# hao-ai-lab/LookaheadDecoding

Measured on NVIDIA H100. Metric: tokens/sec (wall-clock) and accepted-tokens/step, Llama-2-7B W=15 N=5 G=15, higher is better.
Workload: dtype bf16

## Files before the change

### lookaheaddecoding_b200/csrc/attn_mma.cu

```cuda
#include "common.cuh"

namespace lade {

constexpr int ATT_BM = 128;
constexpr int ATT_BN = 64;
constexpr int ATT_STAGES = 3;
constexpr int ATT_THREADS = 256;
constexpr int ATT_RD_SMEM = 1024;
constexpr int ATTN_MAX_COUNTERS = 16384;

__device__ __forceinline__ void cp_async16(void* smem, const void* gmem, int src_bytes) {
  const unsigned s = (unsigned)__cvta_generic_to_shared(smem);
  asm volatile("cp.async.cg.shared.global [%0], [%1], 16, %2;\n" ::"r"(s), "l"(gmem), "r"(src_bytes));
}
__device__ __forceinline__ void cp_async_commit() { asm volatile("cp.async.commit_group;\n" ::); }
template <int N>
__device__ __forceinline__ void cp_async_wait() { asm volatile("cp.async.wait_group %0;\n" ::"n"(N)); }

__device__ __forceinline__ void ldmatrix_x4(unsigned& r0, unsigned& r1, unsigned& r2, unsigned& r3, const void* p) {
  const unsigned a = (unsigned)__cvta_generic_to_shared(p);
  asm volatile("ldmatrix.sync.aligned.m8n8.x4.shared.b16 {%0,%1,%2,%3}, [%4];\n"
               : "=r"(r0), "=r"(r1), "=r"(r2), "=r"(r3) : "r"(a));
}
__device__ __forceinline__ void ldmatrix_x4_trans(unsigned& r0, unsigned& r1, unsigned& r2, unsigned& r3, const void* p) {
  const unsigned a = (unsigned)__cvta_generic_to_shared(p);
  asm volatile("ldmatrix.sync.aligned.m8n8.x4.trans.shared.b16 {%0,%1,%2,%3}, [%4];\n"
               : "=r"(r0), "=r"(r1), "=r"(r2), "=r"(r3) : "r"(a));
}
template <typename T>
__device__ __forceinline__ void mma_16816(float (&c)[4], const unsigned (&a)[4], unsigned b0, unsigned b1);
template <>
__device__ __forceinline__ void mma_16816<__nv_bfloat16>(float (&c)[4], const unsigned (&a)[4], unsigned b0, unsigned b1) {
// ... 314 lines not shown
```

### lookaheaddecoding_b200/csrc/attn_tc.cu

```cuda
#include "tc_common.cuh"

#include <cstdlib>
#include <mutex>
#include <type_traits>
#include <unordered_map>

namespace lade {

constexpr int TC_BM = 128;
constexpr int TC_BN = 128;
constexpr int TC_D = 128;
constexpr int TC_STAGES = 3;
constexpr int TC_CONSUMER_THREADS = 256;
constexpr int TC_THREADS = TC_CONSUMER_THREADS + 32;
constexpr int TC_TILE_BYTES = 128 * 128 * 2;
constexpr int TC_HALF_BYTES = TC_TILE_BYTES / 2;
constexpr int TC_SMEM_TILES = TC_TILE_BYTES * (1 + 2 * TC_STAGES);
constexpr int TC_SMEM_BYTES = TC_SMEM_TILES + 256 + 1024;
constexpr float TC_LOG2E = 1.4426950408889634f;
constexpr int TC_SO_STRIDE = 132;
constexpr int TC_SO_OFFSET = TC_TILE_BYTES;
constexpr int TC_SML_OFFSET = 0;

__device__ long long* g_attn_timing = nullptr;
#define TC_STAMP(slot, tid) do { if (tbuf && threadIdx.x == (tid)) tbuf[slot] = clock64(); } while (0)
enum { TS_START = 0, TS_KFULL0 = 1, TS_SFULL0 = 2, TS_OFINAL = 3, TS_STAGED = 4, TS_CLUSTER = 5, TS_MERGED = 6, TS_END = 7 };

template <typename ET> __device__ __forceinline__ float2 unpack2(uint32_t u);
template <> __device__ __forceinline__ float2 unpack2<__nv_bfloat16>(uint32_t u) {
  return make_float2(__uint_as_float(u << 16), __uint_as_float(u & 0xffff0000u));
}
template <> __device__ __forceinline__ float2 unpack2<__half>(uint32_t u) {
  return __half22float2(*reinterpret_cast<__half2*>(&u));
}

template <typename ET>
__device__ __forceinline__ void qk_tile(float (&s)[64], uint32_t sQ_a, uint32_t sK_a, int wg) {
  wg_fence();
#pragma unroll
  for (int kb = 0; kb < 2; ++kb)
#pragma unroll
    for (int k = 0; k < 4; ++k) {
      const uint64_t da = wg_desc(sQ_a + kb * TC_HALF_BYTES + wg * 8192 + k * 32, 16, 1024);
      const uint64_t db = wg_desc(sK_a + kb * TC_HALF_BYTES + k * 32, 16, 1024);
      wgmma_m64n128_ss<ET>(s, da, db, (kb | k) ? 1u : 0u);
    }
  wg_commit();
  wg_wait_all();
  wg_fence_regs(s);
// ... 9 lines not shown
  wg_wait_all();
  wg_fence_regs(o);
}

__device__ __forceinline__ void tile_mask(uint32_t (&mb)[2][4], const uint32_t* const (&mrow)[2], const int (&row)[2],
                                          int mask_words, int tile0, int kv_len, int q_len, int is_prefill) {
#pragma unroll
  for (int rr = 0; rr < 2; ++rr)
#pragma unroll
    for (int w = 0; w < 4; ++w)
      mb[rr][w] = (tile0 + 32 * w + 32 <= kv_len)
                      ? 0xffffffffu
                      : visible_bits32(mrow[rr], mask_words, tile0 + 32 * w, kv_len, q_len, is_prefill, row[rr]);
}
__device__ __forceinline__ bool vis(const uint32_t (&mb)[2][4], int rr, int i, int e, int t) {
  return (mb[rr][i >> 2] >> (8 * (i & 3) + 2 * t + e)) & 1u;
}

template <typename ET, bool REF>
__global__ void __launch_bounds__(TC_THREADS, 1)
attn_fwd_tc_kernel(const __grid_constant__ CUtensorMap tmQ, const __grid_constant__ CUtensorMap tmK,
                   const __grid_constant__ CUtensorMap tmV, ET* __restrict__ out,
                   const uint32_t* __restrict__ rowmask, int mask_words, const int* __restrict__ meta, int q_pad,
                   int n_heads, int n_kv_heads, int n_splits, float inv_sqrt_d, float2* __restrict__ row_ml) {
  extern __shared__ unsigned char smem_raw[];
  const uint32_t raw_a = smem_u32(smem_raw);
  const uint32_t sQ_a = (raw_a + 1023u) & ~1023u;
  unsigned char* smem = smem_raw + (sQ_a - raw_a);
  const int split = blockIdx.x, h = blockIdx.y, mt = blockIdx.z;
  const int warp = threadIdx.x >> 5, lane = threadIdx.x & 31;

  const int q_len = meta[LADE_M_Q_LEN];
  const int kv_len = meta[LADE_M_KV_LEN];
  const int is_prefill = meta[LADE_M_IS_PREFILL];
  const int T = kv_len + q_len;
  int Tm = T;
  if (is_prefill) Tm = min(T, kv_len + min(q_len, (mt + 1) * TC_BM));
  const int n_tiles = (Tm + TC_BN - 1) / TC_BN;
  const int t_base = n_tiles / n_splits, t_rem = n_tiles - t_base * n_splits;
  const int n_active = n_tiles < n_splits ? n_tiles : n_splits;
  const bool active = split < n_active;
  const int tile_lo = split * t_base + (split < t_rem ? split : t_rem);
  const int my_tiles = active ? t_base + (split < t_rem ? 1 : 0) : 0;
  if (REF && t_base + (t_rem ? 1 : 0) > TC_STAGES) __trap();
  const int hk = h / (n_heads / n_kv_heads);
  const int HD = n_heads * TC_D;
  const long long hm = (long long)h * gridDim.z + mt;
  const int n_wg = (mt * TC_BM + 64 < q_pad) ? 2 : 1;
  const bool zero_last = active && (tile_lo + my_tiles) * TC_BN > T;
  long long* tbuf = g_attn_timing ? g_attn_timing + 16ll * ((blockIdx.z * gridDim.y + blockIdx.y) * gridDim.x + blockIdx.x) : nullptr;
  TC_STAMP(TS_START, 0);
  griddep_launch_dependents();

  uint64_t* bars = reinterpret_cast<uint64_t*>(smem + TC_SMEM_TILES);
  const uint32_t bar0 = smem_u32(bars);
  auto BAR = [&](int i) { return bar0 + 8u * (uint32_t)i; };
  const int B_QFULL = 0, B_KFULL = 1, B_VFULL = 1 + TC_STAGES, B_FREE = 1 + 2 * TC_STAGES, B_VZERO = 1 + 3 * TC_STAGES;
  auto sK_a = [&](int s) { return sQ_a + (uint32_t)TC_TILE_BYTES * (1 + 2 * s); };
  auto sV_a = [&](int s) { return sQ_a + (uint32_t)TC_TILE_BYTES * (2 + 2 * s); };
  auto issue_tile = [&](int j) {
    const int s = j % TC_STAGES;
    const int row0 = (tile_lo + j) * TC_BN;
    mbar_expect_tx(BAR(B_KFULL + s), TC_TILE_BYTES);
    tma_load_3d(sK_a(s), &tmK, BAR(B_KFULL + s), 0, row0, hk);
    tma_load_3d(sK_a(s) + TC_HALF_BYTES, &tmK, BAR(B_KFULL + s), 64, row0, hk);
    mbar_expect_tx(BAR(B_VFULL + s), TC_TILE_BYTES);
    tma_load_3d(sV_a(s), &tmV, BAR(B_VFULL + s), 0, row0, hk);
    tma_load_3d(sV_a(s) + TC_HALF_BYTES, &tmV, BAR(B_VFULL + s), 64, row0, hk);
  };

  if (active && threadIdx.x == TC_CONSUMER_THREADS) {
    mbar_init(BAR(B_QFULL), 1);
    for (int s = 0; s < TC_STAGES; ++s) {
      mbar_init(BAR(B_KFULL + s), 1);
      mbar_init(BAR(B_VFULL + s), 1);
      mbar_init(BAR(B_FREE + s), 4 * n_wg);
    }
    mbar_init(BAR(B_VZERO), 1);
    fence_barrier_init();
    const int n_pre = my_tiles < TC_STAGES ? my_tiles : TC_STAGES;
    int n_old = 0;
    while (n_old < n_pre && (tile_lo + n_old + 1) * TC_BN <= kv_len) ++n_old;
    for (int j = 0; j < n_old; ++j) issue_tile(j);
    griddep_wait();
    mbar_expect_tx(BAR(B_QFULL), TC_TILE_BYTES);
    tma_load_3d(sQ_a, &tmQ, BAR(B_QFULL), 0, mt * TC_BM, h);
    tma_load_3d(sQ_a + TC_HALF_BYTES, &tmQ, BAR(B_QFULL), 64, mt * TC_BM, h);
    for (int j = n_old; j < n_pre; ++j) issue_tile(j);
  }
  __syncthreads();

  const int wg = warp >> 2;
  const int g = lane >> 2, t = lane & 3;
  const int rl[2] = {wg * 64 + (warp & 3) * 16 + g, wg * 64 + (warp & 3) * 16 + g + 8};
  const bool work = active && warp < 8 && wg < n_wg;
  float o[64];
  float m_row[2] = {-INFINITY, -INFINITY}, l_row[2] = {0.f, 0.f};
#pragma unroll
  for (int i = 0; i < 64; ++i) o[i] = 0.f;

  if (warp == 8) {
    if (active) {
      if (lane == 0) {
        for (int j = TC_STAGES; j < my_tiles; ++j) {
          const int s = j % TC_STAGES;
          mbar_wait(BAR(B_FREE + s), ((j / TC_STAGES) - 1) & 1);
          issue_tile(j);
        }
      }
      __syncwarp();
      if (zero_last) {
        const int j = my_tiles - 1, s = j % TC_STAGES;
        const int r0 = T - (tile_lo + j) * TC_BN;
        mbar_wait(BAR(B_VFULL + s), (j / TC_STAGES) & 1);
        unsigned char* pV = smem + TC_TILE_BYTES * (2 + 2 * s);
        const uint4 z = make_uint4(0, 0, 0, 0);
        for (int c = r0 * 8 + lane; c < TC_BN * 8; c += 32) {
          const int r = c >> 3, cc = c & 7;
          *reinterpret_cast<uint4*>(pV + r * 128 + cc * 16) = z;
          *reinterpret_cast<uint4*>(pV + TC_HALF_BYTES + r * 128 + cc * 16) = z;
        }
        fence_proxy_async();
        __syncwarp();
        if (lane == 0) mbar_arrive(BAR(B_VZERO));
      }
    }
    if (REF) {
      cluster_arrive(); cluster_wait();
      cluster_arrive(); cluster_wait();
    }
  } else {
    const int row[2] = {mt * TC_BM + rl[0], mt * TC_BM + rl[1]};
    const uint32_t* const mrow[2] = {
        (row[0] < q_pad && !is_prefill && rowmask != nullptr) ? rowmask + (long long)row[0] * mask_words : nullptr,
        (row[1] < q_pad && !is_prefill && rowmask != nullptr) ? rowmask + (long long)row[1] * mask_words : nullptr};
    auto wait_v = [&](int j) {
      const int s = j % TC_STAGES;
      mbar_wait(BAR(B_VFULL + s), (j / TC_STAGES) & 1);
      if (zero_last && j == my_tiles - 1) mbar_wait(BAR(B_VZERO), 0);
    };
    if (work) mbar_wait(BAR(B_QFULL), 0);
    if (!REF) {
      for (int j = 0; work && j < my_tiles; ++j) {
        const int s = j % TC_STAGES;
        const int tile0 = (tile_lo + j) * TC_BN;
        mbar_wait(BAR(B_KFULL + s), (j / TC_STAGES) & 1);
        if (j == 0) TC_STAMP(TS_KFULL0, 0);
        float sc[64];
        qk_tile<ET>(sc, sQ_a, sK_a(s), wg);
        if (j == 0) TC_STAMP(TS_SFULL0, 0);
        uint32_t mb[2][4];
        tile_mask(mb, mrow, row, mask_words, tile0, kv_len, q_len, is_prefill);
        float off[2];
#pragma unroll
        for (int rr = 0; rr < 2; ++rr) {
          float mx = -INFINITY;
#pragma unroll
          for (int i = 0; i < 16; ++i)
#pragma unroll
            for (int e = 0; e < 2; ++e) mx = fmaxf(mx, vis(mb, rr, i, e, t) ? sc[4 * i + 2 * rr + e] : -INFINITY);
          mx = fmaxf(mx, __shfl_xor_sync(0xffffffffu, mx, 1));
          mx = fmaxf(mx, __shfl_xor_sync(0xffffffffu, mx, 2));
          const float mtile = mx == -INFINITY ? -INFINITY : round_to<ET>(round_to<ET>(mx) * inv_sqrt_d);
          if (mtile > m_row[rr]) {
            const float scale = m_row[rr] == -INFINITY ? 1.f : exp2f((m_row[rr] - mtile) * TC_LOG2E);
            l_row[rr] *= scale;
#pragma unroll
            for (int i = 0; i < 16; ++i) { o[4 * i + 2 * rr] *= scale; o[4 * i + 2 * rr + 1] *= scale; }
            m_row[rr] = mtile;
// ... 9 lines not shown
            round_scale_round2<ET>(sc[4 * i + 2 * rr], sc[4 * i + 2 * rr + 1], inv_sqrt_d, r0, r1);
            const float p0 = vis(mb, rr, i, 0, t) ? ex2_approx(r0 * TC_LOG2E - off[rr]) : 0.f;
            const float p1 = vis(mb, rr, i, 1, t) ? ex2_approx(r1 * TC_LOG2E - off[rr]) : 0.f;
            const uint32_t pk = Elem<ET>::pack2(p0, p1);
            const float2 pr = unpack2<ET>(pk);
            l_row[rr] += pr.x + pr.y;
            pa[4 * (i >> 1) + 2 * (i & 1) + rr] = pk;
          }
        wait_v(j);
        pv_tile<ET>(o, pa, sV_a(s));
        __syncwarp();
        if (lane == 0) mbar_arrive(BAR(B_FREE + s));
      }
#pragma unroll
      for (int rr = 0; rr < 2; ++rr) {
        l_row[rr] += __shfl_xor_sync(0xffffffffu, l_row[rr], 1);
        l_row[rr] += __shfl_xor_sync(0xffffffffu, l_row[rr], 2);
      }
    } else {
      float sc[64];
      uint32_t mb[2][4];
      float mx[2] = {-INFINITY, -INFINITY};
      for (int j = 0; work && j < my_tiles; ++j) {
        mbar_wait(BAR(B_KFULL + j), 0);
        qk_tile<ET>(sc, sQ_a, sK_a(j), wg);
        tile_mask(mb, mrow, row, mask_words, (tile_lo + j) * TC_BN, kv_len, q_len, is_prefill);
#pragma unroll
        for (int rr = 0; rr < 2; ++rr)
#pragma unroll
          for (int i = 0; i < 16; ++i)
#pragma unroll
            for (int e = 0; e < 2; ++e) mx[rr] = fmaxf(mx[rr], vis(mb, rr, i, e, t) ? sc[4 * i + 2 * rr + e] : -INFINITY);
      }
      if (work) {
#pragma unroll
        for (int rr = 0; rr < 2; ++rr) {
          mx[rr] = fmaxf(mx[rr], __shfl_xor_sync(0xffffffffu, mx[rr], 1));
          mx[rr] = fmaxf(mx[rr], __shfl_xor_sync(0xffffffffu, mx[rr], 2));
          const float m_split = mx[rr] == -INFINITY ? -INFINITY : round_to<ET>(round_to<ET>(mx[rr]) * inv_sqrt_d);
          if (t == 0) row_ml[(hm * n_splits + split) * TC_BM + rl[rr]].x = m_split;
        }
      }
      cluster_arrive(); cluster_wait();
      float m_ref[2] = {0.f, 0.f};
      if (work) {
#pragma unroll
        for (int rr = 0; rr < 2; ++rr) {
// ... 37 lines not shown
      }
      cluster_arrive(); cluster_wait();
      float l_all[2] = {0.f, 0.f};
      if (work) {
#pragma unroll
        for (int rr = 0; rr < 2; ++rr)
          for (int sp = 0; sp < n_active; ++sp) l_all[rr] += ld_global_f2(row_ml + (hm * n_splits + sp) * TC_BM + rl[rr]).y;
      }
      for (int j = 0; work && j < my_tiles; ++j) {
        exps(j);
        uint32_t pa[32];
#pragma unroll
        for (int i = 0; i < 16; ++i)
#pragma unroll
          for (int rr = 0; rr < 2; ++rr) {
            const float p0 = l_all[rr] > 0.f ? __fdiv_rn(sc[4 * i + 2 * rr], l_all[rr]) : 0.f;
            const float p1 = l_all[rr] > 0.f ? __fdiv_rn(sc[4 * i + 2 * rr + 1], l_all[rr]) : 0.f;
            pa[4 * (i >> 1) + 2 * (i & 1) + rr] = Elem<ET>::pack2(p0, p1);
          }
        wait_v(j);
        pv_tile<ET>(o, pa, sV_a(j));
      }
    }
    TC_STAMP(TS_OFINAL, 0);
    if (work && n_splits == 1) {
#pragma unroll
      for (int rr = 0; rr < 2; ++rr) {
        if (row[rr] >= q_pad) continue;
        const float inv = REF ? 1.f : (l_row[rr] > 0.f ? 1.f / l_row[rr] : 0.f);
        uint32_t* dst = reinterpret_cast<uint32_t*>(out + (long long)row[rr] * HD + h * TC_D + 2 * t);
#pragma unroll
        for (int i = 0; i < 16; ++i) dst[4 * i] = Elem<ET>::pack2(o[4 * i + 2 * rr] * inv, o[4 * i + 2 * rr + 1] * inv);
      }
    }
  }
  TC_STAMP(TS_STAGED, 0);
  if (n_splits == 1) { TC_STAMP(TS_END, 0); return; }

  const int rows_valid = min(TC_BM, q_pad - mt * TC_BM);
  const int per = (rows_valid + n_active - 1) / n_active;
  cluster_arrive();
  cluster_wait();
  TC_STAMP(TS_CLUSTER, 0);
  int dest[2] = {-1, -1}, r_in[2] = {0, 0};
  if (work) {
#pragma unroll
    for (int rr = 0; rr < 2; ++rr) {
      dest[rr] = rl[rr] < rows_valid ? rl[rr] / per : -2;
      r_in[rr] = rl[rr] - dest[rr] * per;
      if (dest[rr] >= 0 && dest[rr] != split) {
        const int slot = split < dest[rr] ? split : split - 1;
        const uint32_t o_a = dsmem_addr(sQ_a + TC_SO_OFFSET + (uint32_t)(((slot * per + r_in[rr]) * TC_SO_STRIDE + 2 * t) * 4), dest[rr]);
#pragma unroll
        for (int i = 0; i < 16; ++i) st_dsmem_f2(o_a + i * 32, o[4 * i + 2 * rr], o[4 * i + 2 * rr + 1]);
        if (!REF && t == 0)
          st_dsmem_f2(dsmem_addr(sQ_a + TC_SML_OFFSET + (uint32_t)((slot * per + r_in[rr]) * 8), dest[rr]), m_row[rr], l_row[rr]);
      }
    }
  }
  cluster_arrive();
  cluster_wait();
  TC_STAMP(TS_MERGED, 0);
  if (work) {
    const float2* sml = reinterpret_cast<const float2*>(smem + TC_SML_OFFSET);
    const float* so = reinterpret_cast<const float*>(smem + TC_SO_OFFSET);
#pragma unroll
    for (int rr = 0; rr < 2; ++rr) {
      if (dest[rr] != split) continue;
      float inv = 1.f;
      if (!REF) {
        float mmax = m_row[rr];
        for (int k = 0; k < n_active - 1; ++k) mmax = fmaxf(mmax, sml[k * per + r_in[rr]].x);
        float wgt = (m_row[rr] == -INFINITY) ? 0.f : exp2f((m_row[rr] - mmax) * TC_LOG2E);
        float lsum = l_row[rr] * wgt;
#pragma unroll
        for (int i = 0; i < 16; ++i) { o[4 * i + 2 * rr] *= wgt; o[4 * i + 2 * rr + 1] *= wgt; }
        for (int k = 0; k < n_active - 1; ++k) {
          const float2 ml = sml[k * per + r_in[rr]];
          wgt = (ml.x == -INFINITY) ? 0.f : exp2f((ml.x - mmax) * TC_LOG2E);
          lsum += ml.y * wgt;
          const float* src = so + (k * per + r_in[rr]) * TC_SO_STRIDE + 2 * t;
#pragma unroll
          for (int i = 0; i < 16; ++i) {
            const float2 x = *reinterpret_cast<const float2*>(src + 8 * i);
            o[4 * i + 2 * rr] += x.x * wgt;
            o[4 * i + 2 * rr + 1] += x.y * wgt;
          }
        }
        inv = lsum > 0.f ? 1.f / lsum : 0.f;
      } else {
        for (int k = 0; k < n_active - 1; ++k) {
          const float* src = so + (k * per + r_in[rr]) * TC_SO_STRIDE + 2 * t;
#pragma unroll
          for (int i = 0; i < 16; ++i) {
            const float2 x = *reinterpret_cast<const float2*>(src + 8 * i);
            o[4 * i + 2 * rr] += x.x;
            o[4 * i + 2 * rr + 1] += x.y;
          }
        }
      }
      const int row = mt * TC_BM + rl[rr];
      if (row < q_pad) {
        uint32_t* dst = reinterpret_cast<uint32_t*>(out + (long long)row * HD + h * TC_D + 2 * t);
#pragma unroll
        for (int i = 0; i < 16; ++i) dst[4 * i] = Elem<ET>::pack2(o[4 * i + 2 * rr] * inv, o[4 * i + 2 * rr + 1] * inv);
      }
    }
  }
  TC_STAMP(TS_END, 0);
}

int attn_tc_set_timing_buffer(void* dev_ptr) {
  long long* p = reinterpret_cast<long long*>(dev_ptr);
  cudaError_t e = cudaMemcpyToSymbol(g_attn_timing, &p, sizeof(p));
  if (e != cudaSuccess) { set_cuda_error(e, "cudaMemcpyToSymbol(g_attn_timing)"); return LADE_ECUDA; }
  return LADE_OK;
}

EncodeTiledFn get_encode_fn() {
  static EncodeTiledFn fn = nullptr;
  static bool tried = false;
  if (!tried) {
    tried = true;
    void* p = nullptr;
    cudaDriverEntryPointQueryResult qres;
    if (cudaGetDriverEntryPoint("cuTensorMapEncodeTiled", &p, cudaEnableDefault, &qres) == cudaSuccess &&
        qres == cudaDriverEntryPointSuccess)
      fn = reinterpret_cast<EncodeTiledFn>(p);
  }
  return fn;
}

// ... 44 lines not shown
  return v != 0;
}

template <typename ET, bool REF>
static int launch_tc(cudaStream_t stream, const void* q, const void* k_cache, const void* v_cache, void* out,
                     const uint32_t* rowmask, int mask_words, const int32_t* meta, void* scratch, int q_pad, int n_heads,
                     int n_kv_heads, int head_dim, int kv_capacity, int n_splits) {
  const int q_tiles = (q_pad + TC_BM - 1) / TC_BM;
  if ((reinterpret_cast<uintptr_t>(q) & 15) || (reinterpret_cast<uintptr_t>(k_cache) & 15) ||
      (reinterpret_cast<uintptr_t>(v_cache) & 15))
    return LADE_EINVAL;
  CUtensorMap tmQ, tmK, tmV;
  int rc;
  if ((rc = get_tensor_map(q, q_pad, n_heads, &tmQ)) != LADE_OK) return rc;
  if ((rc = get_tensor_map(k_cache, kv_capacity, n_kv_heads, &tmK)) != LADE_OK) return rc;
  if ((rc = get_tensor_map(v_cache, kv_capacity, n_kv_heads, &tmV)) != LADE_OK) return rc;
  static unsigned long long attr_devs = 0;
  int cur_dev = 0;
  LADE_CUDA_CHECK(cudaGetDevice(&cur_dev));
  if (!((attr_devs >> (cur_dev & 63)) & 1ull)) {
    LADE_CUDA_CHECK(cudaFuncSetAttribute(attn_fwd_tc_kernel<ET, REF>, cudaFuncAttributeMaxDynamicSharedMemorySize, TC_SMEM_BYTES));
    attr_devs |= 1ull << (cur_dev & 63);
  }
  cudaLaunchConfig_t cfg = {};
  cfg.gridDim = dim3(n_splits, n_heads, q_tiles);
  cfg.blockDim = dim3(TC_THREADS);
  cfg.dynamicSmemBytes = TC_SMEM_BYTES;
  cfg.stream = stream;
  cudaLaunchAttribute attr[2];
  attr[0].id = cudaLaunchAttributeClusterDimension;
  attr[0].val.clusterDim.x = n_splits;
  attr[0].val.clusterDim.y = 1;
  attr[0].val.clusterDim.z = 1;
  attr[1].id = cudaLaunchAttributeProgrammaticStreamSerialization;
  attr[1].val.programmaticStreamSerializationAllowed = 1;
  cfg.attrs = attr;
  cfg.numAttrs = pdl_enabled() ? 2 : 1;
  const float inv_sqrt_d = 1.0f / sqrtf((float)head_dim);
  float* part_o = reinterpret_cast<float*>(reinterpret_cast<char*>(scratch) + 65536);
  float2* row_ml = reinterpret_cast<float2*>(part_o + (size_t)n_splits * n_heads * q_tiles * TC_BM * TC_D);
  cudaError_t e = cudaLaunchKernelEx(&cfg, attn_fwd_tc_kernel<ET, REF>, tmQ, tmK, tmV, (ET*)out, rowmask, mask_words, meta,
                                     q_pad, n_heads, n_kv_heads, n_splits, inv_sqrt_d, row_ml);
  if (e != cudaSuccess) { set_cuda_error(e, "cudaLaunchKernelEx(attn_fwd_tc_kernel)"); return LADE_ECUDA; }
  return LADE_OK;
}

template <typename ET>
static int attn_fwd_tc_launch_t(cudaStream_t stream, const void* q, const void* k_cache, const void* v_cache, void* out,
                                const uint32_t* rowmask, int mask_words, const int32_t* meta, void* scratch, int q_pad,
                                int n_heads, int n_kv_heads, int head_dim, int kv_capacity, int kv_bound, int n_splits) {
  (void)kv_bound;
  if (head_dim != TC_D) return LADE_EUNSUPPORTED;
  if (n_splits > 8) n_splits = 8;
  return launch_tc<ET, false>(stream, q, k_cache, v_cache, out, rowmask, mask_words, meta, scratch, q_pad, n_heads,
                              n_kv_heads, head_dim, kv_capacity, n_splits);
}

int attn_fwd_tc_launch(cudaStream_t stream, const void* q, const void* k_cache, const void* v_cache, void* out,
                       const uint32_t* rowmask, int mask_words, const int32_t* meta, void* scratch, int q_pad, int n_heads,
                       int n_kv_heads, int head_dim, int kv_capacity, int kv_bound, int n_splits, int is_f16) {
  if (is_f16)
    return attn_fwd_tc_launch_t<__half>(stream, q, k_cache, v_cache, out, rowmask, mask_words, meta, scratch, q_pad, n_heads,
                                        n_kv_heads, head_dim, kv_capacity, kv_bound, n_splits);
  return attn_fwd_tc_launch_t<__nv_bfloat16>(stream, q, k_cache, v_cache, out, rowmask, mask_words, meta, scratch, q_pad,
                                             n_heads, n_kv_heads, head_dim, kv_capacity, kv_bound, n_splits);
}

template <typename ET>
static int attn_fwd_tc_exact_launch_t(cudaStream_t stream, const void* q, const void* k_cache, const void* v_cache, void* out,
                                      const uint32_t* rowmask, int mask_words, const int32_t* meta, void* scratch, int q_pad,
                                      int n_heads, int n_kv_heads, int head_dim, int kv_capacity, int kv_bound, int n_splits) {
  if (head_dim != TC_D) return LADE_EUNSUPPORTED;
  if (n_splits > 8) n_splits = 8;
  if (kv_bound < 1 || (kv_bound + TC_BN - 1) / TC_BN > TC_STAGES * n_splits) {
    set_error_string("lade_attn_fwd impl 3: kv_bound exceeds 384 * n_splits (every K/V tile of a split must stay in shared memory)");
    return LADE_EUNSUPPORTED;
  }
  return launch_tc<ET, true>(stream, q, k_cache, v_cache, out, rowmask, mask_words, meta, scratch, q_pad, n_heads,
                             n_kv_heads, head_dim, kv_capacity, n_splits);
}

int attn_fwd_tc_exact_launch(cudaStream_t stream, const void* q, const void* k_cache, const void* v_cache, void* out,
                             const uint32_t* rowmask, int mask_words, const int32_t* meta, void* scratch, int q_pad, int n_heads,
                             int n_kv_heads, int head_dim, int kv_capacity, int kv_bound, int n_splits, int is_f16) {
  if (is_f16)
    return attn_fwd_tc_exact_launch_t<__half>(stream, q, k_cache, v_cache, out, rowmask, mask_words, meta, scratch, q_pad,
                                              n_heads, n_kv_heads, head_dim, kv_capacity, kv_bound, n_splits);
  return attn_fwd_tc_exact_launch_t<__nv_bfloat16>(stream, q, k_cache, v_cache, out, rowmask, mask_words, meta, scratch, q_pad,
                                                   n_heads, n_kv_heads, head_dim, kv_capacity, kv_bound, n_splits);
}

}
```

### lookaheaddecoding_b200/csrc/common.cuh

```cuda
#pragma once
#include <cuda_runtime.h>
#include <cuda_bf16.h>
#include <cuda_fp16.h>
#include <stdint.h>
#include "../../include/lade_sm100.h"

namespace lade {

void set_cuda_error(cudaError_t e, const char* where);
void set_error_string(const char* msg);

#define LADE_CUDA_CHECK(expr)                                   \
  do {                                                          \
    cudaError_t _e = (expr);                                    \
    if (_e != cudaSuccess) {                                    \
      ::lade::set_cuda_error(_e, #expr);                        \
      return LADE_ECUDA;                                        \
    }                                                           \
  } while (0)

#define LADE_LAUNCH_CHECK(name)                                 \
  do {                                                          \
    cudaError_t _e = cudaGetLastError();                        \
    if (_e != cudaSuccess) {                                    \
      ::lade::set_cuda_error(_e, name);                         \
      return LADE_ECUDA;                                        \
    }                                                           \
  } while (0)

__host__ __device__ inline int rowdesc_make(int cls, int blk, int idx) {
// ... 75 lines not shown
```

### lookaheaddecoding_b200/csrc/gemm_tc.cu

```cuda
#include "tc_common.cuh"

#include <mutex>
#include <unordered_map>

namespace lade {

constexpr int GM_THREADS = 288;
constexpr int GM_PRODUCER = 256;
constexpr int GM_BK = 64;
constexpr int GM_A_BYTES = 128 * GM_BK * 2;
constexpr int GM_MAX_STAGES = 11;
constexpr int GM_SMEM_LIMIT = 227 * 1024;
constexpr int GM_BAR_BYTES = 8 * (2 * GM_MAX_STAGES + 2);

__device__ __forceinline__ void tma_load_2d(uint32_t dst, const CUtensorMap* tm, uint32_t bar, int c0, int c1) {
  asm volatile(
      "cp.async.bulk.tensor.2d.shared::cluster.global.mbarrier::complete_tx::bytes [%0], [%1, {%3, %4}], [%2];"
      ::"r"(dst), "l"(reinterpret_cast<uint64_t>(tm)), "r"(bar), "r"(c0), "r"(c1) : "memory");
}

__device__ long long* g_gemm_timing = nullptr;
__device__ __forceinline__ long long globaltimer_ns() {
  long long t;
  asm volatile("mov.u64 %0, %globaltimer;" : "=l"(t));
  return t;
}
#define GM_STAMP(slot, tid) do { if (tbuf && threadIdx.x == (tid)) tbuf[slot] = globaltimer_ns(); } while (0)

template <int SK>
__device__ __forceinline__ void reduce_splits(__nv_bfloat16* __restrict__ C, uint32_t smem_base, int BN, int M, int N, int ldc,
                                              int n0, int y) {
  constexpr int ITEMS = 16 / SK;
  const int rows_per = 128 / SK;
  const int r0 = y * rows_per;
  const int c4n = BN >> 2;
  const int total = rows_per * c4n;
  uint32_t peer_base[SK];
#pragma unroll
  for (int p = 0; p < SK; ++p) peer_base[p] = dsmem_addr(smem_base, (uint32_t)p);
  for (int i0 = threadIdx.x; i0 < total; i0 += ITEMS * GM_THREADS) {
    float4 v[ITEMS][SK];
#pragma unroll
    for (int it = 0; it < ITEMS; ++it) {
      const int i = i0 + it * GM_THREADS;
      if (i < total) {
        const int r = r0 + i / c4n;
        const int c4 = i - (i / c4n) * c4n;
        const uint32_t off = (uint32_t)((r * (BN + 4) + c4 * 4) * 4);
#pragma unroll
// ... 309 lines not shown
```

### lookaheaddecoding_b200/csrc/tc_common.cuh

```cuda
#pragma once
#include "common.cuh"

#include <cuda.h>
#include <type_traits>

namespace lade {

__device__ __forceinline__ uint32_t smem_u32(const void* p) { return (uint32_t)__cvta_generic_to_shared(p); }

__device__ __forceinline__ void mbar_init(uint32_t bar, uint32_t count) {
  asm volatile("mbarrier.init.shared::cta.b64 [%0], %1;" ::"r"(bar), "r"(count));
}
__device__ __forceinline__ void mbar_expect_tx(uint32_t bar, uint32_t bytes) {
  asm volatile("mbarrier.arrive.expect_tx.shared::cta.b64 _, [%0], %1;" ::"r"(bar), "r"(bytes) : "memory");
}
__device__ __forceinline__ void mbar_arrive(uint32_t bar) {
  asm volatile("mbarrier.arrive.shared::cta.b64 _, [%0];" ::"r"(bar) : "memory");
}
__device__ __forceinline__ bool mbar_try_wait(uint32_t bar, uint32_t parity) {
  uint32_t ok;
  asm volatile(
      "{\n\t.reg .pred p;\n\t"
      "mbarrier.try_wait.parity.shared::cta.b64 p, [%1], %2;\n\t"
      "selp.u32 %0, 1, 0, p;\n\t}"
      : "=r"(ok) : "r"(bar), "r"(parity) : "memory");
  return ok != 0;
}
__device__ __forceinline__ void mbar_wait(uint32_t bar, uint32_t parity) {
  if (mbar_try_wait(bar, parity)) return;
  const long long t0 = clock64();
  while (!mbar_try_wait(bar, parity)) {
    if (clock64() - t0 > 4000000000LL) __trap();
  }
}
__device__ __forceinline__ void fence_barrier_init() { asm volatile("fence.mbarrier_init.release.cluster;" ::: "memory"); }
__device__ __forceinline__ void fence_proxy_async() { asm volatile("fence.proxy.async.shared::cta;" ::: "memory"); }

__device__ __forceinline__ void tma_load_3d(uint32_t dst, const CUtensorMap* tm, uint32_t bar, int c0, int c1, int c2) {
  asm volatile(
      "cp.async.bulk.tensor.3d.shared::cluster.global.mbarrier::complete_tx::bytes [%0], [%1, {%3, %4, %5}], [%2];"
      ::"r"(dst), "l"(reinterpret_cast<uint64_t>(tm)), "r"(bar), "r"(c0), "r"(c1), "r"(c2) : "memory");
}
__device__ __forceinline__ void tma_prefetch_desc(const CUtensorMap* tm) {
  asm volatile("prefetch.tensormap [%0];" ::"l"(reinterpret_cast<uint64_t>(tm)) : "memory");
}

__device__ __forceinline__ uint64_t wg_desc(uint32_t saddr, uint32_t lbo_bytes, uint32_t sbo_bytes) {
  uint64_t d = 0;
  d |= (uint64_t)((saddr & 0x3FFFF) >> 4);
  d |= (uint64_t)((lbo_bytes >> 4) & 0x3FFF) << 16;
  d |= (uint64_t)((sbo_bytes >> 4) & 0x3FFF) << 32;
  d |= (uint64_t)1 << 62;
  return d;
}
__device__ __forceinline__ void wg_fence() { asm volatile("wgmma.fence.sync.aligned;" ::: "memory"); }
// ... 73 lines not shown
  return *reinterpret_cast<unsigned*>(&v);
}

__device__ __forceinline__ void griddep_wait() { asm volatile("griddepcontrol.wait;" ::: "memory"); }
__device__ __forceinline__ void griddep_launch_dependents() { asm volatile("griddepcontrol.launch_dependents;" ::: "memory"); }

__device__ __forceinline__ void cluster_arrive() { asm volatile("barrier.cluster.arrive.release.aligned;" ::: "memory"); }
__device__ __forceinline__ void cluster_wait() { asm volatile("barrier.cluster.wait.acquire.aligned;" ::: "memory"); }
__device__ __forceinline__ uint32_t dsmem_addr(uint32_t local_smem_addr, uint32_t cta_rank) {
  uint32_t r;
  asm volatile("mapa.shared::cluster.u32 %0, %1, %2;" : "=r"(r) : "r"(local_smem_addr), "r"(cta_rank));
  return r;
}
__device__ __forceinline__ float4 ld_dsmem_f4(uint32_t addr) {
  float4 v;
  asm volatile("ld.shared::cluster.v4.f32 {%0, %1, %2, %3}, [%4];" : "=f"(v.x), "=f"(v.y), "=f"(v.z), "=f"(v.w) : "r"(addr));
  return v;
}
__device__ __forceinline__ float4 ld_global_f4(const float* p) {
  float4 v;
  asm volatile("ld.global.cg.v4.f32 {%0, %1, %2, %3}, [%4];" : "=f"(v.x), "=f"(v.y), "=f"(v.z), "=f"(v.w) : "l"(p));
  return v;
}
__device__ __forceinline__ float2 ld_global_f2(const float2* p) {
  float2 v;
  asm volatile("ld.global.cg.v2.f32 {%0, %1}, [%2];" : "=f"(v.x), "=f"(v.y) : "l"(p));
  return v;
}
__device__ __forceinline__ void st_dsmem_f4(uint32_t addr, float a, float b, float c, float d) {
  asm volatile("st.shared::cluster.v4.f32 [%0], {%1, %2, %3, %4};" ::"r"(addr), "f"(a), "f"(b), "f"(c), "f"(d) : "memory");
}
__device__ __forceinline__ void st_dsmem_f2(uint32_t addr, float a, float b) {
  asm volatile("st.shared::cluster.v2.f32 [%0], {%1, %2};" ::"r"(addr), "f"(a), "f"(b) : "memory");
}
__device__ __forceinline__ float2 ld_dsmem_f2(uint32_t addr) {
  float2 v;
  asm volatile("ld.shared::cluster.v2.f32 {%0, %1}, [%2];" : "=f"(v.x), "=f"(v.y) : "r"(addr));
  return v;
}


typedef CUresult (*EncodeTiledFn)(CUtensorMap*, CUtensorMapDataType, cuuint32_t, void*, const cuuint64_t*, const cuuint64_t*,
                                  const cuuint32_t*, const cuuint32_t*, CUtensorMapInterleave, CUtensorMapSwizzle,
                                  CUtensorMapL2promotion, CUtensorMapFloatOOBfill);
EncodeTiledFn get_encode_fn();

}
```

Baseline: 114.7.

## Replace cluster DSMEM split merge with last-block global merge and register reallocation

```diff
diff --git a/lookaheaddecoding_b200/csrc/attn_mma.cu b/lookaheaddecoding_b200/csrc/attn_mma.cu
--- a/lookaheaddecoding_b200/csrc/attn_mma.cu
+++ b/lookaheaddecoding_b200/csrc/attn_mma.cu
@@ -7,7 +7,6 @@
 constexpr int ATT_STAGES = 3;
 constexpr int ATT_THREADS = 256;
 constexpr int ATT_RD_SMEM = 1024;
-constexpr int ATTN_MAX_COUNTERS = 16384;
 
 __device__ __forceinline__ void cp_async16(void* smem, const void* gmem, int src_bytes) {
   const unsigned s = (unsigned)__cvta_generic_to_shared(smem);
diff --git a/lookaheaddecoding_b200/csrc/attn_tc.cu b/lookaheaddecoding_b200/csrc/attn_tc.cu
--- a/lookaheaddecoding_b200/csrc/attn_tc.cu
+++ b/lookaheaddecoding_b200/csrc/attn_tc.cu
@@ -12,19 +12,23 @@
 constexpr int TC_D = 128;
 constexpr int TC_STAGES = 3;
 constexpr int TC_CONSUMER_THREADS = 256;
-constexpr int TC_THREADS = TC_CONSUMER_THREADS + 32;
+constexpr int TC_THREADS = TC_CONSUMER_THREADS + 128;
+constexpr int TC_CONSUMER_REGS = 232;
+constexpr int TC_PRODUCER_REGS = 40;
+static_assert(TC_CONSUMER_THREADS * TC_CONSUMER_REGS + (TC_THREADS - TC_CONSUMER_THREADS) * TC_PRODUCER_REGS <= 65536,
+              "register budget exceeds the register file");
 constexpr int TC_TILE_BYTES = 128 * 128 * 2;
 constexpr int TC_HALF_BYTES = TC_TILE_BYTES / 2;
 constexpr int TC_SMEM_TILES = TC_TILE_BYTES * (1 + 2 * TC_STAGES);
 constexpr int TC_SMEM_BYTES = TC_SMEM_TILES + 256 + 1024;
 constexpr float TC_LOG2E = 1.4426950408889634f;
-constexpr int TC_SO_STRIDE = 132;
-constexpr int TC_SO_OFFSET = TC_TILE_BYTES;
-constexpr int TC_SML_OFFSET = 0;
+constexpr int TC_MAX_SPLITS = 8;
+constexpr int TC_MG_STRIDE = TC_D + 8;
+constexpr int TC_MG_ML_OFFSET = TC_SMEM_TILES - TC_MAX_SPLITS * TC_BM * 8;
 
 __device__ long long* g_attn_timing = nullptr;
-#define TC_STAMP(slot, tid) do { if (tbuf && threadIdx.x == (tid)) tbuf[slot] = clock64(); } while (0)
-enum { TS_START = 0, TS_KFULL0 = 1, TS_SFULL0 = 2, TS_OFINAL = 3, TS_STAGED = 4, TS_CLUSTER = 5, TS_MERGED = 6, TS_END = 7 };
+#define TC_STAMP(slot, tid) do { if (tbuf && threadIdx.x == (tid)) tbuf[slot] = globaltimer_ns(); } while (0)
+enum { TS_START = 0, TS_KFULL0 = 1, TS_SFULL0 = 2, TS_OFINAL = 3, TS_STAGED = 4, TS_ARRIVED = 5, TS_END = 7 };
 
 template <typename ET> __device__ __forceinline__ float2 unpack2(uint32_t u);
 template <> __device__ __forceinline__ float2 unpack2<__nv_bfloat16>(uint32_t u) {
@@ -80,7 +84,9 @@
 attn_fwd_tc_kernel(const __grid_constant__ CUtensorMap tmQ, const __grid_constant__ CUtensorMap tmK,
                    const __grid_constant__ CUtensorMap tmV, ET* __restrict__ out,
                    const uint32_t* __restrict__ rowmask, int mask_words, const int* __restrict__ meta, int q_pad,
-                   int n_heads, int n_kv_heads, int n_splits, float inv_sqrt_d, float2* __restrict__ row_ml) {
+                   int n_heads, int n_kv_heads, int n_splits, float inv_sqrt_d, float2* __restrict__ row_ml,
+                   float* __restrict__ part_o, int* __restrict__ counters) {
+  __shared__ int s_last;
   extern __shared__ unsigned char smem_raw[];
   const uint32_t raw_a = smem_u32(smem_raw);
   const uint32_t sQ_a = (raw_a + 1023u) & ~1023u;
@@ -109,11 +115,13 @@
   long long* tbuf = g_attn_timing ? g_attn_timing + 16ll * ((blockIdx.z * gridDim.y + blockIdx.y) * gridDim.x + blockIdx.x) : nullptr;
   TC_STAMP(TS_START, 0);
   griddep_launch_dependents();
+  if (!REF && !active) return;
 
   uint64_t* bars = reinterpret_cast<uint64_t*>(smem + TC_SMEM_TILES);
   const uint32_t bar0 = smem_u32(bars);
   auto BAR = [&](int i) { return bar0 + 8u * (uint32_t)i; };
-  const int B_QFULL = 0, B_KFULL = 1, B_VFULL = 1 + TC_STAGES, B_FREE = 1 + 2 * TC_STAGES, B_VZERO = 1 + 3 * TC_STAGES;
+  const int B_QFULL = 0, B_KFULL = 1, B_VFULL = 1 + TC_STAGES, B_FREE = 1 + 2 * TC_STAGES, B_VZERO = 1 + 3 * TC_STAGES,
+            B_DONE = 2 + 3 * TC_STAGES;
   auto sK_a = [&](int s) { return sQ_a + (uint32_t)TC_TILE_BYTES * (1 + 2 * s); };
   auto sV_a = [&](int s) { return sQ_a + (uint32_t)TC_TILE_BYTES * (2 + 2 * s); };
   auto issue_tile = [&](int j) {
@@ -135,6 +143,7 @@
       mbar_init(BAR(B_FREE + s), 4 * n_wg);
     }
     mbar_init(BAR(B_VZERO), 1);
+    mbar_init(BAR(B_DONE), 4 * n_wg);
     fence_barrier_init();
     const int n_pre = my_tiles < TC_STAGES ? my_tiles : TC_STAGES;
     int n_old = 0;
@@ -148,17 +157,9 @@
   }
   __syncthreads();
 
-  const int wg = warp >> 2;
-  const int g = lane >> 2, t = lane & 3;
-  const int rl[2] = {wg * 64 + (warp & 3) * 16 + g, wg * 64 + (warp & 3) * 16 + g + 8};
-  const bool work = active && warp < 8 && wg < n_wg;
-  float o[64];
-  float m_row[2] = {-INFINITY, -INFINITY}, l_row[2] = {0.f, 0.f};
-#pragma unroll
-  for (int i = 0; i < 64; ++i) o[i] = 0.f;
-
-  if (warp == 8) {
-    if (active) {
+  if (warp >= 8) {
+    setmaxnreg_dec<TC_PRODUCER_REGS>();
+    if (warp == 8 && active) {
       if (lane == 0) {
         for (int j = TC_STAGES; j < my_tiles; ++j) {
           const int s = j % TC_STAGES;
@@ -182,27 +183,44 @@
         __syncwarp();
         if (lane == 0) mbar_arrive(BAR(B_VZERO));
       }
+      if (REF) {
+        mbar_wait(BAR(B_QFULL), 0);
+        for (int j = 0; j < my_tiles; ++j) {
+          mbar_wait(BAR(B_KFULL + j), 0);
+          mbar_wait(BAR(B_VFULL + j), 0);
+        }
+      }
     }
     if (REF) {
       cluster_arrive(); cluster_wait();
       cluster_arrive(); cluster_wait();
     }
+    if (warp == 8 && active) mbar_wait(BAR(B_DONE), 0);
   } else {
+    setmaxnreg_inc<TC_CONSUMER_REGS>();
+    const int wg = warp >> 2;
+    const int g = lane >> 2, t = lane & 3;
+    const int rl[2] = {wg * 64 + (warp & 3) * 16 + g, wg * 64 + (warp & 3) * 16 + g + 8};
+    const bool work = active && wg < n_wg;
+    float o[64];
+    float m_row[2] = {-INFINITY, -INFINITY}, l_row[2] = {0.f, 0.f};
+#pragma unroll
+    for (int i = 0; i < 64; ++i) o[i] = 0.f;
     const int row[2] = {mt * TC_BM + rl[0], mt * TC_BM + rl[1]};
     const uint32_t* const mrow[2] = {
         (row[0] < q_pad && !is_prefill && rowmask != nullptr) ? rowmask + (long long)row[0] * mask_words : nullptr,
         (row[1] < q_pad && !is_prefill && rowmask != nullptr) ? rowmask + (long long)row[1] * mask_words : nullptr};
     auto wait_v = [&](int j) {
       const int s = j % TC_STAGES;
-      mbar_wait(BAR(B_VFULL + s), (j / TC_STAGES) & 1);
-      if (zero_last && j == my_tiles - 1) mbar_wait(BAR(B_VZERO), 0);
+      mbar_wait_unbounded(BAR(B_VFULL + s), (j / TC_STAGES) & 1);
+      if (zero_last && j == my_tiles - 1) mbar_wait_unbounded(BAR(B_VZERO), 0);
     };
-    if (work) mbar_wait(BAR(B_QFULL), 0);
+    if (work) mbar_wait_unbounded(BAR(B_QFULL), 0);
     if (!REF) {
       for (int j = 0; work && j < my_tiles; ++j) {
         const int s = j % TC_STAGES;
         const int tile0 = (tile_lo + j) * TC_BN;
-        mbar_wait(BAR(B_KFULL + s), (j / TC_STAGES) & 1);
+        mbar_wait_unbounded(BAR(B_KFULL + s), (j / TC_STAGES) & 1);
         if (j == 0) TC_STAMP(TS_KFULL0, 0);
         float sc[64];
         qk_tile<ET>(sc, sQ_a, sK_a(s), wg);
@@ -258,7 +276,7 @@
       uint32_t mb[2][4];
       float mx[2] = {-INFINITY, -INFINITY};
       for (int j = 0; work && j < my_tiles; ++j) {
-        mbar_wait(BAR(B_KFULL + j), 0);
+        mbar_wait_unbounded(BAR(B_KFULL + j), 0);
         qk_tile<ET>(sc, sQ_a, sK_a(j), wg);
         tile_mask(mb, mrow, row, mask_words, (tile_lo + j) * TC_BN, kv_len, q_len, is_prefill);
 #pragma unroll
@@ -342,92 +360,134 @@
         pv_tile<ET>(o, pa, sV_a(j));
       }
     }
+    if (work) {
+      __syncwarp();
+      if (lane == 0) mbar_arrive(BAR(B_DONE));
+    }
     TC_STAMP(TS_OFINAL, 0);
-    if (work && n_splits == 1) {
+    if (n_splits == 1) {
+      if (work) {
+#pragma unroll
+        for (int rr = 0; rr < 2; ++rr) {
+          if (row[rr] >= q_pad) continue;
+          const float inv = REF ? 1.f : (l_row[rr] > 0.f ? 1.f / l_row[rr] : 0.f);
+          uint32_t* dst = reinterpret_cast<uint32_t*>(out + (long long)row[rr] * HD + h * TC_D + 2 * t);
+#pragma unroll
+          for (int i = 0; i < 16; ++i) dst[4 * i] = Elem<ET>::pack2(o[4 * i + 2 * rr] * inv, o[4 * i + 2 * rr + 1] * inv);
+        }
+      }
+      TC_STAMP(TS_END, 0);
+      return;
+    }
+    if (!active) return;
+
+    griddep_wait();
+    const int rows_valid = min(TC_BM, q_pad - mt * TC_BM);
+    const int per = (rows_valid + n_active - 1) / n_active;
+    float* const po = part_o + hm * n_splits * TC_BM * TC_D;
+    float2* const ml = row_ml + hm * n_splits * TC_BM;
+    if (work) {
 #pragma unroll
       for (int rr = 0; rr < 2; ++rr) {
-        if (row[rr] >= q_pad) continue;
-        const float inv = REF ? 1.f : (l_row[rr] > 0.f ? 1.f / l_row[rr] : 0.f);
+        if (rl[rr] >= rows_valid) continue;
+        float* dst = po + ((long long)split * TC_BM + rl[rr]) * TC_D + 2 * t;
+#pragma unroll
+        for (int i = 0; i < 16; ++i)
+          *reinterpret_cast<float2*>(dst + 8 * i) = make_float2(o[4 * i + 2 * rr], o[4 * i + 2 * rr + 1]);
+        if (!REF && t == 0) ml[split * TC_BM + rl[rr]] = make_float2(m_row[rr], l_row[rr]);
+      }
+    }
+    TC_STAMP(TS_STAGED, 0);
+    __threadfence();
+    named_bar_sync(1, TC_CONSUMER_THREADS);
+    if (threadIdx.x == 0) {
+      s_last = atomicAdd(counters + hm, 1) == n_active - 1;
+      if (s_last) counters[hm] = 0;
+    }
+    named_bar_sync(1, TC_CONSUMER_THREADS);
+    TC_STAMP(TS_ARRIVED, 0);
+    if (!s_last) return;
+    __threadfence();
+    const int n_other = n_active - 1;
+    float* const stage = reinterpret_cast<float*>(smem);
+    const float2* const sml = reinterpret_cast<const float2*>(smem + TC_MG_ML_OFFSET);
+    const int chunk = n_other ? min(rows_valid, TC_MG_ML_OFFSET / (n_other * TC_MG_STRIDE * 4)) : rows_valid;
+    if (!REF) {
+      for (int c = threadIdx.x; c < n_active * (TC_BM / 2); c += TC_CONSUMER_THREADS)
+        cp_async_cg16(smem + TC_MG_ML_OFFSET + 16 * c, ml + 2 * c);
+    }
+    for (int r0 = 0; r0 < rows_valid; r0 += chunk) {
+      const int nr = min(chunk, rows_valid - r0);
+      for (int slot = 0; slot < n_other; ++slot) {
+        const float* src = po + ((long long)(slot < split ? slot : slot + 1) * TC_BM + r0) * TC_D;
+        float* dst = stage + slot * chunk * TC_MG_STRIDE;
+        for (int c = threadIdx.x; c < nr * (TC_D / 4); c += TC_CONSUMER_THREADS)
+          cp_async_cg16(dst + (c >> 5) * TC_MG_STRIDE + 4 * (c & 31), src + 4 * c);
+      }
+      cp_async_wait_all();
+      named_bar_sync(1, TC_CONSUMER_THREADS);
+#pragma unroll
+      for (int rr = 0; work && rr < 2; ++rr) {
+        if (rl[rr] < r0 || rl[rr] >= r0 + nr) continue;
+        const int d = rl[rr] / per;
+        auto part = [&](int k, int i) -> float2 {
+          return k == split ? make_float2(o[4 * i + 2 * rr], o[4 * i + 2 * rr + 1])
+                            : *reinterpret_cast<const float2*>(stage + ((k < split ? k : k - 1) * chunk + rl[rr] - r0) * TC_MG_STRIDE + 2 * t + 8 * i);
+        };
+        float a[32];
+        float inv = 1.f;
+        if (!REF) {
+          float mmax = -INFINITY;
+          for (int k = 0; k < n_active; ++k) mmax = fmaxf(mmax, sml[k * TC_BM + rl[rr]].x);
+          const float2 mld = sml[d * TC_BM + rl[rr]];
+          float wgt = (mld.x == -INFINITY) ? 0.f : exp2f((mld.x - mmax) * TC_LOG2E);
+          float lsum = __fmul_rn(mld.y, wgt);
+#pragma unroll
+          for (int i = 0; i < 16; ++i) {
+            const float2 x = part(d, i);
+            a[2 * i] = __fmul_rn(x.x, wgt);
+            a[2 * i + 1] = __fmul_rn(x.y, wgt);
+          }
+          for (int k = 0; k < n_active; ++k) {
+            if (k == d) continue;
+            const float2 v = sml[k * TC_BM + rl[rr]];
+            wgt = (v.x == -INFINITY) ? 0.f : exp2f((v.x - mmax) * TC_LOG2E);
+            lsum = __fmaf_rn(v.y, wgt, lsum);
+#pragma unroll
+            for (int i = 0; i < 16; ++i) {
+              const float2 x = part(k, i);
+              a[2 * i] = __fmaf_rn(x.x, wgt, a[2 * i]);
+              a[2 * i + 1] = __fmaf_rn(x.y, wgt, a[2 * i + 1]);
+            }
+          }
+          inv = lsum > 0.f ? 1.f / lsum : 0.f;
+        } else {
+#pragma unroll
+          for (int i = 0; i < 16; ++i) {
+            const float2 x = part(d, i);
+            a[2 * i] = x.x;
+            a[2 * i + 1] = x.y;
+          }
+          for (int k = 0; k < n_active; ++k) {
+            if (k == d) continue;
+#pragma unroll
+            for (int i = 0; i < 16; ++i) {
+              const float2 x = part(k, i);
+              a[2 * i] = __fadd_rn(a[2 * i], x.x);
+              a[2 * i + 1] = __fadd_rn(a[2 * i + 1], x.y);
+            }
+          }
+        }
         uint32_t* dst = reinterpret_cast<uint32_t*>(out + (long long)row[rr] * HD + h * TC_D + 2 * t);
 #pragma unroll
-        for (int i = 0; i < 16; ++i) dst[4 * i] = Elem<ET>::pack2(o[4 * i + 2 * rr] * inv, o[4 * i + 2 * rr + 1] * inv);
-      }
-    }
-  }
-  TC_STAMP(TS_STAGED, 0);
-  if (n_splits == 1) { TC_STAMP(TS_END, 0); return; }
-
-  const int rows_valid = min(TC_BM, q_pad - mt * TC_BM);
-  const int per = (rows_valid + n_active - 1) / n_active;
-  cluster_arrive();
-  cluster_wait();
-  TC_STAMP(TS_CLUSTER, 0);
-  int dest[2] = {-1, -1}, r_in[2] = {0, 0};
-  if (work) {
-#pragma unroll
-    for (int rr = 0; rr < 2; ++rr) {
-      dest[rr] = rl[rr] < rows_valid ? rl[rr] / per : -2;
-      r_in[rr] = rl[rr] - dest[rr] * per;
-      if (dest[rr] >= 0 && dest[rr] != split) {
-        const int slot = split < dest[rr] ? split : split - 1;
-        const uint32_t o_a = dsmem_addr(sQ_a + TC_SO_OFFSET + (uint32_t)(((slot * per + r_in[rr]) * TC_SO_STRIDE + 2 * t) * 4), dest[rr]);
-#pragma unroll
-        for (int i = 0; i < 16; ++i) st_dsmem_f2(o_a + i * 32, o[4 * i + 2 * rr], o[4 * i + 2 * rr + 1]);
-        if (!REF && t == 0)
-          st_dsmem_f2(dsmem_addr(sQ_a + TC_SML_OFFSET + (uint32_t)((slot * per + r_in[rr]) * 8), dest[rr]), m_row[rr], l_row[rr]);
-      }
-    }
-  }
-  cluster_arrive();
-  cluster_wait();
-  TC_STAMP(TS_MERGED, 0);
-  if (work) {
-    const float2* sml = reinterpret_cast<const float2*>(smem + TC_SML_OFFSET);
-    const float* so = reinterpret_cast<const float*>(smem + TC_SO_OFFSET);
-#pragma unroll
-    for (int rr = 0; rr < 2; ++rr) {
-      if (dest[rr] != split) continue;
-      float inv = 1.f;
-      if (!REF) {
-        float mmax = m_row[rr];
-        for (int k = 0; k < n_active - 1; ++k) mmax = fmaxf(mmax, sml[k * per + r_in[rr]].x);
-        float wgt = (m_row[rr] == -INFINITY) ? 0.f : exp2f((m_row[rr] - mmax) * TC_LOG2E);
-        float lsum = l_row[rr] * wgt;
-#pragma unroll
-        for (int i = 0; i < 16; ++i) { o[4 * i + 2 * rr] *= wgt; o[4 * i + 2 * rr + 1] *= wgt; }
-        for (int k = 0; k < n_active - 1; ++k) {
-          const float2 ml = sml[k * per + r_in[rr]];
-          wgt = (ml.x == -INFINITY) ? 0.f : exp2f((ml.x - mmax) * TC_LOG2E);
-          lsum += ml.y * wgt;
-          const float* src = so + (k * per + r_in[rr]) * TC_SO_STRIDE + 2 * t;
-#pragma unroll
-          for (int i = 0; i < 16; ++i) {
-            const float2 x = *reinterpret_cast<const float2*>(src + 8 * i);
-            o[4 * i + 2 * rr] += x.x * wgt;
-            o[4 * i + 2 * rr + 1] += x.y * wgt;
-          }
-        }
-        inv = lsum > 0.f ? 1.f / lsum : 0.f;
-      } else {
-        for (int k = 0; k < n_active - 1; ++k) {
-          const float* src = so + (k * per + r_in[rr]) * TC_SO_STRIDE + 2 * t;
-#pragma unroll
-          for (int i = 0; i < 16; ++i) {
-            const float2 x = *reinterpret_cast<const float2*>(src + 8 * i);
-            o[4 * i + 2 * rr] += x.x;
-            o[4 * i + 2 * rr + 1] += x.y;
-          }
-        }
-      }
-      const int row = mt * TC_BM + rl[rr];
-      if (row < q_pad) {
-        uint32_t* dst = reinterpret_cast<uint32_t*>(out + (long long)row * HD + h * TC_D + 2 * t);
-#pragma unroll
-        for (int i = 0; i < 16; ++i) dst[4 * i] = Elem<ET>::pack2(o[4 * i + 2 * rr] * inv, o[4 * i + 2 * rr + 1] * inv);
-      }
-    }
-  }
-  TC_STAMP(TS_END, 0);
+        for (int i = 0; i < 16; ++i)
+          dst[4 * i] = REF ? Elem<ET>::pack2(a[2 * i], a[2 * i + 1])
+                           : Elem<ET>::pack2(__fmul_rn(a[2 * i], inv), __fmul_rn(a[2 * i + 1], inv));
+      }
+      named_bar_sync(1, TC_CONSUMER_THREADS);
+    }
+    TC_STAMP(TS_END, 0);
+  }
 }
 
 int attn_tc_set_timing_buffer(void* dev_ptr) {
@@ -518,25 +578,34 @@
     LADE_CUDA_CHECK(cudaFuncSetAttribute(attn_fwd_tc_kernel<ET, REF>, cudaFuncAttributeMaxDynamicSharedMemorySize, TC_SMEM_BYTES));
     attr_devs |= 1ull << (cur_dev & 63);
   }
+  if (n_splits > 1 && (long long)n_heads * q_tiles > ATTN_MAX_COUNTERS) return LADE_EUNSUPPORTED;
   cudaLaunchConfig_t cfg = {};
   cfg.gridDim = dim3(n_splits, n_heads, q_tiles);
   cfg.blockDim = dim3(TC_THREADS);
   cfg.dynamicSmemBytes = TC_SMEM_BYTES;
   cfg.stream = stream;
   cudaLaunchAttribute attr[2];
-  attr[0].id = cudaLaunchAttributeClusterDimension;
-  attr[0].val.clusterDim.x = n_splits;
-  attr[0].val.clusterDim.y = 1;
-  attr[0].val.clusterDim.z = 1;
-  attr[1].id = cudaLaunchAttributeProgrammaticStreamSerialization;
-  attr[1].val.programmaticStreamSerializationAllowed = 1;
+  int n_attr = 0;
+  if (pdl_enabled()) {
+    attr[n_attr].id = cudaLaunchAttributeProgrammaticStreamSerialization;
+    attr[n_attr].val.programmaticStreamSerializationAllowed = 1;
+    ++n_attr;
+  }
+  if (REF) {
+    attr[n_attr].id = cudaLaunchAttributeClusterDimension;
+    attr[n_attr].val.clusterDim.x = n_splits;
+    attr[n_attr].val.clusterDim.y = 1;
+    attr[n_attr].val.clusterDim.z = 1;
+    ++n_attr;
+  }
   cfg.attrs = attr;
-  cfg.numAttrs = pdl_enabled() ? 2 : 1;
+  cfg.numAttrs = n_attr;
   const float inv_sqrt_d = 1.0f / sqrtf((float)head_dim);
-  float* part_o = reinterpret_cast<float*>(reinterpret_cast<char*>(scratch) + 65536);
+  int* counters = reinterpret_cast<int*>(scratch);
+  float* part_o = reinterpret_cast<float*>(counters + ATTN_MAX_COUNTERS);
   float2* row_ml = reinterpret_cast<float2*>(part_o + (size_t)n_splits * n_heads * q_tiles * TC_BM * TC_D);
   cudaError_t e = cudaLaunchKernelEx(&cfg, attn_fwd_tc_kernel<ET, REF>, tmQ, tmK, tmV, (ET*)out, rowmask, mask_words, meta,
-                                     q_pad, n_heads, n_kv_heads, n_splits, inv_sqrt_d, row_ml);
+                                     q_pad, n_heads, n_kv_heads, n_splits, inv_sqrt_d, row_ml, part_o, counters);
   if (e != cudaSuccess) { set_cuda_error(e, "cudaLaunchKernelEx(attn_fwd_tc_kernel)"); return LADE_ECUDA; }
   return LADE_OK;
 }
@@ -547,7 +616,7 @@
                                 int n_heads, int n_kv_heads, int head_dim, int kv_capacity, int kv_bound, int n_splits) {
   (void)kv_bound;
   if (head_dim != TC_D) return LADE_EUNSUPPORTED;
-  if (n_splits > 8) n_splits = 8;
+  if (n_splits > TC_MAX_SPLITS) n_splits = TC_MAX_SPLITS;
   return launch_tc<ET, false>(stream, q, k_cache, v_cache, out, rowmask, mask_words, meta, scratch, q_pad, n_heads,
                               n_kv_heads, head_dim, kv_capacity, n_splits);
 }
@@ -567,7 +636,7 @@
                                       const uint32_t* rowmask, int mask_words, const int32_t* meta, void* scratch, int q_pad,
                                       int n_heads, int n_kv_heads, int head_dim, int kv_capacity, int kv_bound, int n_splits) {
   if (head_dim != TC_D) return LADE_EUNSUPPORTED;
-  if (n_splits > 8) n_splits = 8;
+  if (n_splits > TC_MAX_SPLITS) n_splits = TC_MAX_SPLITS;
   if (kv_bound < 1 || (kv_bound + TC_BN - 1) / TC_BN > TC_STAGES * n_splits) {
     set_error_string("lade_attn_fwd impl 3: kv_bound exceeds 384 * n_splits (every K/V tile of a split must stay in shared memory)");
     return LADE_EUNSUPPORTED;
diff --git a/lookaheaddecoding_b200/csrc/common.cuh b/lookaheaddecoding_b200/csrc/common.cuh
--- a/lookaheaddecoding_b200/csrc/common.cuh
+++ b/lookaheaddecoding_b200/csrc/common.cuh
@@ -6,6 +6,8 @@
 #include "../../include/lade_sm100.h"
 
 namespace lade {
+
+constexpr int ATTN_MAX_COUNTERS = 16384;
 
 void set_cuda_error(cudaError_t e, const char* where);
 void set_error_string(const char* msg);
diff --git a/lookaheaddecoding_b200/csrc/gemm_tc.cu b/lookaheaddecoding_b200/csrc/gemm_tc.cu
--- a/lookaheaddecoding_b200/csrc/gemm_tc.cu
+++ b/lookaheaddecoding_b200/csrc/gemm_tc.cu
@@ -20,11 +20,6 @@
 }
 
 __device__ long long* g_gemm_timing = nullptr;
-__device__ __forceinline__ long long globaltimer_ns() {
-  long long t;
-  asm volatile("mov.u64 %0, %globaltimer;" : "=l"(t));
-  return t;
-}
 #define GM_STAMP(slot, tid) do { if (tbuf && threadIdx.x == (tid)) tbuf[slot] = globaltimer_ns(); } while (0)
 
 template <int SK>
diff --git a/lookaheaddecoding_b200/csrc/tc_common.cuh b/lookaheaddecoding_b200/csrc/tc_common.cuh
--- a/lookaheaddecoding_b200/csrc/tc_common.cuh
+++ b/lookaheaddecoding_b200/csrc/tc_common.cuh
@@ -31,6 +31,10 @@
   const long long t0 = clock64();
   while (!mbar_try_wait(bar, parity)) {
     if (clock64() - t0 > 4000000000LL) __trap();
+  }
+}
+__device__ __forceinline__ void mbar_wait_unbounded(uint32_t bar, uint32_t parity) {
+  while (!mbar_try_wait(bar, parity)) {
   }
 }
 __device__ __forceinline__ void fence_barrier_init() { asm volatile("fence.mbarrier_init.release.cluster;" ::: "memory"); }
@@ -150,21 +154,23 @@
   asm volatile("ld.global.cg.v4.f32 {%0, %1, %2, %3}, [%4];" : "=f"(v.x), "=f"(v.y), "=f"(v.z), "=f"(v.w) : "l"(p));
   return v;
 }
+__device__ __forceinline__ void cp_async_cg16(void* smem, const void* gmem) {
+  asm volatile("cp.async.cg.shared.global [%0], [%1], 16;" ::"r"(smem_u32(smem)), "l"(gmem) : "memory");
+}
+__device__ __forceinline__ void cp_async_wait_all() { asm volatile("cp.async.wait_all;" ::: "memory"); }
 __device__ __forceinline__ float2 ld_global_f2(const float2* p) {
   float2 v;
   asm volatile("ld.global.cg.v2.f32 {%0, %1}, [%2];" : "=f"(v.x), "=f"(v.y) : "l"(p));
   return v;
 }
-__device__ __forceinline__ void st_dsmem_f4(uint32_t addr, float a, float b, float c, float d) {
-  asm volatile("st.shared::cluster.v4.f32 [%0], {%1, %2, %3, %4};" ::"r"(addr), "f"(a), "f"(b), "f"(c), "f"(d) : "memory");
-}
-__device__ __forceinline__ void st_dsmem_f2(uint32_t addr, float a, float b) {
-  asm volatile("st.shared::cluster.v2.f32 [%0], {%1, %2};" ::"r"(addr), "f"(a), "f"(b) : "memory");
-}
-__device__ __forceinline__ float2 ld_dsmem_f2(uint32_t addr) {
-  float2 v;
-  asm volatile("ld.shared::cluster.v2.f32 {%0, %1}, [%2];" : "=f"(v.x), "=f"(v.y) : "r"(addr));
-  return v;
+
+template <uint32_t N> __device__ __forceinline__ void setmaxnreg_inc() { asm volatile("setmaxnreg.inc.sync.aligned.u32 %0;" ::"n"(N)); }
+template <uint32_t N> __device__ __forceinline__ void setmaxnreg_dec() { asm volatile("setmaxnreg.dec.sync.aligned.u32 %0;" ::"n"(N)); }
+
+__device__ __forceinline__ long long globaltimer_ns() {
+  long long t;
+  asm volatile("mov.u64 %0, %globaltimer;" : "=l"(t));
+  return t;
 }
 
 
```

Result: faster. 122.3 (median of 6 runs) (+6.6%).
